# jianzhnie/ScaleRL

Measured on NVIDIA H100. Metric: learner_frames_per_sec, higher is better.
Workload: dtype bf16

## Files before the change

scalerl_b200/csrc/common.cuh:

```cuda
#pragma once
#include <cuda_runtime.h>
#include <cuda_bf16.h>
#include <stdint.h>
#include "wgmma.cuh"

#define SRL_DEVINL __device__ __forceinline__

#ifndef SRL_SPIN_LIMIT
#define SRL_SPIN_LIMIT (1u << 24)
#endif

namespace srl {

SRL_DEVINL uint32_t smem_u32(const void* p) { return static_cast<uint32_t>(__cvta_generic_to_shared(p)); }

SRL_DEVINL void mbar_init(uint64_t* bar, uint32_t count) {
  asm volatile("mbarrier.init.shared::cta.b64 [%0], %1;" ::"r"(smem_u32(bar)), "r"(count) : "memory");
}
SRL_DEVINL void mbar_fence_init() { asm volatile("fence.mbarrier_init.release.cluster;" ::: "memory"); }
SRL_DEVINL void mbar_arrive(uint64_t* bar) {
  asm volatile("{\n\t.reg .b64 st;\n\tmbarrier.arrive.shared::cta.b64 st, [%0];\n\t}" ::"r"(smem_u32(bar)) : "memory");
}
SRL_DEVINL void mbar_arrive_expect_tx(uint64_t* bar, uint32_t bytes) {
  asm volatile("{\n\t.reg .b64 st;\n\tmbarrier.arrive.expect_tx.shared::cta.b64 st, [%0], %1;\n\t}" ::"r"(smem_u32(bar)), "r"(bytes)
// ... 111 lines not shown

SRL_DEVINL uint64_t make_smem_desc(uint32_t saddr, uint32_t lbo_bytes, uint32_t sbo_bytes) {
  uint64_t d = 0;
  d |= (uint64_t)((saddr & 0x3FFFF) >> 4);
  d |= (uint64_t)((lbo_bytes >> 4) & 0x3FFF) << 16;
  d |= (uint64_t)((sbo_bytes >> 4) & 0x3FFF) << 32;
  d |= (uint64_t)1 << 62;
  return d;
}
SRL_DEVINL uint64_t make_smem_desc_sw64(uint32_t saddr, uint32_t lbo_bytes, uint32_t sbo_bytes) {
  return (make_smem_desc(saddr, lbo_bytes, sbo_bytes) & ~((uint64_t)3 << 62)) | ((uint64_t)2 << 62);
}

SRL_DEVINL uint32_t swz128(uint32_t row, uint32_t chunk) { return row * 128u + ((chunk ^ (row & 7u)) << 4); }
SRL_DEVINL uint32_t swz64(uint32_t row, uint32_t chunk) { return row * 64u + ((chunk ^ ((row >> 1) & 3u)) << 4); }

SRL_DEVINL uint32_t pack_bf16x2(float lo, float hi) {
  __nv_bfloat162 v = __floats2bfloat162_rn(lo, hi);
  return *reinterpret_cast<uint32_t*>(&v);
}
SRL_DEVINL float bf16_lo(uint32_t v) { return __uint_as_float(v << 16); }
SRL_DEVINL float bf16_hi(uint32_t v) { return __uint_as_float(v & 0xFFFF0000u); }

SRL_DEVINL void red_add_v4(float* addr, float a, float b, float c, float d) {
  asm volatile("red.global.add.v4.f32 [%0], {%1, %2, %3, %4};" ::"l"(addr), "f"(a), "f"(b), "f"(c), "f"(d) : "memory");
}
SRL_DEVINL void red_add_16(float* dst, const float (&v)[16], float scale = 1.0f) {
#pragma unroll
  for (int j = 0; j < 16; j += 4) red_add_v4(dst + j, v[j] * scale, v[j + 1] * scale, v[j + 2] * scale, v[j + 3] * scale);
}

SRL_DEVINL int ld_action(const int64_t* p, int A) {
  const long long a = __ldg(reinterpret_cast<const long long*>(p));
  return a < 0 ? 0 : (a >= A ? A - 1 : (int)a);
}

SRL_DEVINL uint4 philox4x32_10(uint4 c, uint2 k) {
#pragma unroll
  for (int r = 0; r < 10; ++r) {
    const uint32_t hi0 = __umulhi(0xD2511F53u, c.x), lo0 = 0xD2511F53u * c.x;
    const uint32_t hi1 = __umulhi(0xCD9E8D57u, c.z), lo1 = 0xCD9E8D57u * c.z;
    c = make_uint4(hi1 ^ c.y ^ k.x, lo1, hi0 ^ c.w ^ k.y, lo0);
    k.x += 0x9E3779B9u; k.y += 0xBB67AE85u;
  }
  return c;
}
// ... 14 lines not shown
```

scalerl_b200/csrc/encoder.cu:

```cuda
#include "encoder_problems.cuh"
#include "tma_problems.cuh"
#include "res_problems.cuh"
#include "enc_fused.cuh"
#include "kernels.h"
#include <stdio.h>
#include <stdlib.h>

namespace srl {

constexpr int PACK_BLOCKS_FK = 256, PACK_BLOCKS_FD = 256, PACK_BLOCKS_CONV = 288;
SRL_DEVINL void pack_store(bf16* __restrict__ out, bf16* __restrict__ out_lo, int64_t i, float v) {
  const bf16 hi = __float2bfloat16_rn(v);
  out[i] = hi;
  if (out_lo) out_lo[i] = __float2bfloat16_rn(v - __bfloat162float(hi));
}
SRL_DEVINL void pack_store2(bf16* __restrict__ out, bf16* __restrict__ out_lo, int64_t i, float v0, float v1) {
  const bf16 h0 = __float2bfloat16_rn(v0), h1 = __float2bfloat16_rn(v1);
  *reinterpret_cast<uint32_t*>(out + i) = pack_bf16x2(v0, v1);
  if (out_lo) *reinterpret_cast<uint32_t*>(out_lo + i) = pack_bf16x2(v0 - __bfloat162float(h0), v1 - __bfloat162float(h1));
}
__global__ void __launch_bounds__(256) pack_weights_kernel(ParamPtrs p, bf16* __restrict__ out, bf16* __restrict__ out_lo, int skip_w1k) {
  pdl_wait(2);
  __shared__ __align__(16) float tile[64 * 99];
  const int t = threadIdx.x, b = blockIdx.x;
// ... 303 lines not shown
                            const StepStreams& S, bool fused_front) {
  if (frames <= 0) return cudaSuccess;
  if ((mode != 0 && mode != 1) || !maps.valid) return cudaErrorInvalidValue;
  const int sp = mode;
  if (sp && !buf.lo.wpack) return cudaErrorInvalidValue;
  const cudaStream_t st = S.main;
  if (fused_front && !sp && (reinterpret_cast<uintptr_t>(obs) & 15) == 0) {
    EncFusedParams q{obs, p.w1, p.b1, p.w2, p.b2, buf.xs, buf.hi.a1, buf.hi.a2, frames, buf.NF};
    S.b(PS_ENC_FUSED); SRL_TRY(enc_fused_fwd_launch(q, kPersistentCtas, st)); S.e(PS_ENC_FUSED);
    SRL_TRY(S.join(LANE_PACK));
  } else {
  S.b(PS_S2D); SRL_TRY(launch_s2d(obs, frames, buf.xs, st, p.w1, buf.hi.wpack + WPack::W1K, sp ? buf.lo.wpack + WPack::W1K : nullptr)); S.e(PS_S2D);
  { RConv1Fwd::Params q{maps.xs_w, maps.hi.w1k, maps.lo.w1k, p.b1, buf.hi.a1, buf.lo.a1, frames, buf.NF};
    S.b(PS_CONV1_FWD); SRL_TRY(res_fwd_launch<RConv1Fwd>(q, cdiv(frames * 441, 128), kPersistentCtas, st, sp)); S.e(PS_CONV1_FWD); }
  SRL_TRY(S.join(LANE_PACK));
  { RConv2Fwd::Params q{maps.hi.a1p0_w, maps.hi.a1p1_w, maps.hi.w2k, maps.lo.a1p0_w, maps.lo.a1p1_w, maps.lo.w2k, p.b2, buf.hi.a2, buf.lo.a2, frames};
    S.b(PS_CONV2_FWD); SRL_TRY(res_fwd_launch<RConv2Fwd>(q, cdiv(frames * 100, 128), kPersistentCtas, st, sp)); S.e(PS_CONV2_FWD); }
  }
  { RConv3Fwd::Params q{maps.hi.a2_w, maps.hi.w3k, maps.lo.a2_w, maps.lo.w3k, p.b3, buf.hi.a3, buf.lo.a3, frames};
    S.b(PS_CONV3_FWD); SRL_TRY(res_fwd_launch<RConv3Fwd>(q, cdiv(frames * 81, 128), kPersistentCtas, st, sp)); S.e(PS_CONV3_FWD); }
  { TFcFwd::Params q{maps.hi.a3m128, maps.hi.wfk, maps.lo.a3m128, maps.lo.wfk, buf.hpart, frames};
    static_assert(TFcFwd::SPLITS == FC_SPLITS, "split count");
    S.b(PS_FC_FWD);
    if (sp) SRL_TRY((igemm_tma_launch<TFcFwd, 1>(q, dim3(cdiv(frames, 128), 8 * FC_SPLITS), st)));
    else SRL_TRY((igemm_tma_launch<TFcFwd, 0>(q, dim3(cdiv(frames, 128), 8 * FC_SPLITS), st)));
    S.e(PS_FC_FWD); }
  return cudaSuccess;
}

cudaError_t encoder_backward(int frames, const EncoderBuffers& buf, const ParamPtrs& g, const TmaMaps& maps, int mode,
                             const StepStreams& S, BwdParts parts, bool a3t_done) {
  if (frames <= 0) return cudaSuccess;
  if ((mode != 0 && mode != 1) || !maps.valid) return cudaErrorInvalidValue;
  const int sp = mode;
  if (sp && !buf.lo.wpack) return cudaErrorInvalidValue;
  const bool do_fc = parts & BWD_FC, do_conv = parts & BWD_CONV;
  const cudaStream_t st = S.main, s1 = S.lane(LANE_FC_WGRAD), s2 = S.lane(LANE_CONV3_WGRAD), s3 = S.lane(LANE_CONV2_WGRAD);
  if (do_fc) {
    SRL_TRY(S.fork(LANE_FC_WGRAD));
    { const bool native = !sp && buf.a3t != nullptr;
      S.b(PS_FC_WGRAD);
      if (native) {
        if (!a3t_done) SRL_TRY(launch_a3_transpose(buf.hi.a3, buf.a3t, frames, s1));
        TFcWgradN::Params q{maps.hi.dhm64, maps.a3tm64, g.wf, g.bf, frames};
        SRL_TRY((igemm_tma_launch<TFcWgradN, 0>(q, dim3(1, 4 * (TFcWgradN::NCT + 1)), s1)));
      } else {
        TFcWgrad::Params q{maps.hi.dhm64, maps.hi.a3m64, maps.lo.dhm64, maps.lo.a3m64, g.wf, g.bf, frames};
        if (sp) SRL_TRY((igemm_tma_launch<TFcWgrad, 1>(q, dim3(1, 4 * 50), s1))); else SRL_TRY((igemm_tma_launch<TFcWgrad, 0>(q, dim3(1, 4 * 50), s1)));
      }
      S.e(PS_FC_WGRAD); }
    { TFcDgrad::Params q{maps.hi.dhm128, maps.hi.wfd, maps.lo.dhm128, maps.lo.wfd, buf.hi.a3, buf.hi.da3, buf.lo.da3, frames};
      S.b(PS_FC_DGRAD);
      if (sp) SRL_TRY((igemm_tma_launch<TFcDgrad, 1>(q, dim3(cdiv(frames, 128), 49), st))); else SRL_TRY((igemm_tma_launch<TFcDgrad, 0>(q, dim3(cdiv(frames, 128), 49), st)));
      S.e(PS_FC_DGRAD); }
    if (!do_conv) SRL_TRY(S.join(LANE_FC_WGRAD));
  }
  if (!do_conv) return cudaSuccess;
  SRL_TRY(S.fork(LANE_CONV3_WGRAD));
  float* part3 = buf.wgrad_part;
  float* part2 = part3 + (size_t)WG_PART_CTAS * WSP_W3;
  float* part1 = part2 + (size_t)WG_PART_CTAS * WSP_W2;
  int n3 = 0, n2 = 0, n1 = 0;
  { RConv3Wgrad::Params q{maps.hi.a2_w, maps.hi.da3g_b, maps.lo.a2_w, maps.lo.da3g_b, part3, frames * 81, 0};
    S.b(PS_CONV3_WGRAD); SRL_TRY(res_wgrad_launch<RConv3Wgrad>(q, side_wgrad_ctas(), s2, &n3, sp)); S.e(PS_CONV3_WGRAD); }
  if (!S.collapsed) SRL_TRY(launch_wgrad_reduce<WgradReduce3>(part3, n3, g.w3, g.b3, s2));
  { RConv3Dgrad::Params q{maps.hi.da3g_w, maps.hi.w3d, maps.lo.da3g_w, maps.lo.w3d, buf.hi.a2, buf.hi.da2, buf.lo.da2, frames};
    S.b(PS_CONV3_DGRAD); SRL_TRY(res_fwd_launch<RConv3Dgrad>(q, cdiv(frames * 81, 128), bwd_ctas(), st, sp)); S.e(PS_CONV3_DGRAD); }
  SRL_TRY(S.fork(LANE_CONV2_WGRAD));
  { RConv2Wgrad::Params q{maps.hi.a1p0_w, maps.hi.a1p1_w, maps.hi.da2g_b, maps.lo.a1p0_w, maps.lo.a1p1_w, maps.lo.da2g_b, part2, frames * 100, 0};
    S.b(PS_CONV2_WGRAD); SRL_TRY(res_wgrad_launch<RConv2Wgrad>(q, side_wgrad_ctas(), s3, &n2, sp)); S.e(PS_CONV2_WGRAD); }
  if (!S.collapsed) SRL_TRY(launch_wgrad_reduce<WgradReduce2>(part2, n2, g.w2, g.b2, s3));
  { RConv2Dgrad::Params q{maps.hi.da2g_w, maps.hi.w2d, maps.lo.da2g_w, maps.lo.w2d, buf.hi.a1, buf.hi.da1, buf.lo.da1, frames, buf.NF};
    S.b(PS_CONV2_DGRAD); SRL_TRY(res_fwd_launch<RConv2Dgrad>(q, cdiv(frames * 100, 128), bwd_ctas(), st, sp)); S.e(PS_CONV2_DGRAD); }
  { RConv1Wgrad::Params q{maps.xs_w, maps.hi.da1g_b, maps.lo.da1g_b, part1, frames * 441, 0};
    S.b(PS_CONV1_WGRAD); SRL_TRY(res_wgrad_launch<RConv1Wgrad>(q, bwd_ctas(), st, &n1, sp)); S.e(PS_CONV1_WGRAD); }
  S.b(PS_WGRAD_FINALIZE);
// ... 14 lines not shown
```

scalerl_b200/csrc/igemm_res.cuh:

```cuda
#pragma once
#include "igemm_tma.cuh"

namespace srl {

constexpr int RES_THREADS = 384;
constexpr int RES_PRODUCER_REGS = 40, RES_CONSUMER_REGS = 232;
constexpr int RES_MAX_TAPS = 10;


template <int N, int ROWB, class F>
SRL_DEVINL void wg_acc_stage_bf16(const float (&d)[2][N / 2], uint8_t* buf, int wt, int bar, F f) {
  static_assert(ROWB % 16 == 0 && ROWB >= 2 * N, "16-byte aligned rows that hold N bf16");
  const int w = wt >> 5, l = wt & 31;
  named_bar(bar, 128);
#pragma unroll
  for (int h = 0; h < 2; ++h)
#pragma unroll
    for (int i = 0; i < N / 2; i += 2) {
      const int row = 64 * h + 16 * w + (l >> 2) + 8 * ((i >> 1) & 1), col = 8 * (i >> 2) + 2 * (l & 3);
      *reinterpret_cast<uint32_t*>(buf + row * ROWB + col * 2) = pack_bf16x2(f(col, d[h][i]), f(col + 1, d[h][i + 1]));
    }
  named_bar(bar, 128);
}
template <class P, int SPLIT>
struct ResFwdCfg {
  static constexpr int ALO = (SPLIT && P::A_LO) ? 1 : 0;
  static constexpr int WIN_BYTES = ((P::WROWS * 128 + 1023) / 1024) * 1024;
  static constexpr int IN_HI_BYTES = P::NWIN * WIN_BYTES;
  static constexpr int IN_BYTES = IN_HI_BYTES * (1 + ALO);
  static constexpr int W_HI_BYTES = P::NT * P::BN * 128;
  static constexpr int W_BYTES = W_HI_BYTES * (1 + SPLIT);
  static constexpr bool TILE_EPI = P::TILE_ROWB > 0 && !SPLIT;
  static constexpr int TILE_IMG_BYTES = 128 * P::TILE_ROWB > WG_IMG_BYTES ? 128 * P::TILE_ROWB : WG_IMG_BYTES;
  static constexpr bool IMG1 = !TILE_EPI && W_BYTES + IN_BYTES + 2 * WG_IMG_BYTES + 1024 + 256 > 232448;
  static constexpr int IMG_BYTES = TILE_EPI ? TILE_IMG_BYTES : IMG1 ? WG_IMG_BYTES / 2 : WG_IMG_BYTES;
  static constexpr int FIT = fit_stages(SPLIT ? P::SPLIT_STAGES : P::STAGES, W_BYTES + 2 * IMG_BYTES + 1024 + 256, IN_BYTES);
  static constexpr int STAGES = FIT > 1 ? FIT & ~1 : 1;
  static constexpr int SMEM_BYTES = W_BYTES + STAGES * IN_BYTES + 2 * IMG_BYTES + 1024 + 256;
  static_assert(SMEM_BYTES <= 232448, "shared memory budget (227 KB)");
  static_assert(W_BYTES % 1024 == 0, "weight block alignment");
  static_assert(P::BN == 32 || P::BN == 64 || P::BN == 128, "MMA N");
};

template <class P, int SPLIT>
__global__ void __launch_bounds__(RES_THREADS, 1) res_fwd_kernel(const __grid_constant__ typename P::Params p) {
  using C = ResFwdCfg<P, SPLIT>;
// ... 362 lines not shown
```

scalerl_b200/csrc/igemm_tma.cuh:

```cuda
#pragma once
#include <cuda.h>
#include "common.cuh"
#include "kernels.h"

namespace srl {

SRL_DEVINL void tma_prefetch_desc(const CUtensorMap* m) {
  asm volatile("prefetch.tensormap [%0];" ::"l"(reinterpret_cast<uint64_t>(m)) : "memory");
}
SRL_DEVINL void tma_load_2d(void* dst, const CUtensorMap* m, uint64_t* bar, int c0, int c1) {
  asm volatile("cp.async.bulk.tensor.2d.shared::cluster.global.mbarrier::complete_tx::bytes [%0], [%1, {%3, %4}], [%2];"
               ::"r"(smem_u32(dst)), "l"(reinterpret_cast<uint64_t>(m)), "r"(smem_u32(bar)), "r"(c0), "r"(c1) : "memory");
}
SRL_DEVINL void tma_load_3d(void* dst, const CUtensorMap* m, uint64_t* bar, int c0, int c1, int c2) {
  asm volatile("cp.async.bulk.tensor.3d.shared::cluster.global.mbarrier::complete_tx::bytes [%0], [%1, {%3, %4, %5}], [%2];"
               ::"r"(smem_u32(dst)), "l"(reinterpret_cast<uint64_t>(m)), "r"(smem_u32(bar)), "r"(c0), "r"(c1), "r"(c2) : "memory");
}
SRL_DEVINL void tma_load_4d(void* dst, const CUtensorMap* m, uint64_t* bar, int c0, int c1, int c2, int c3) {
  asm volatile("cp.async.bulk.tensor.4d.shared::cluster.global.mbarrier::complete_tx::bytes [%0], [%1, {%3, %4, %5, %6}], [%2];"
               ::"r"(smem_u32(dst)), "l"(reinterpret_cast<uint64_t>(m)), "r"(smem_u32(bar)), "r"(c0), "r"(c1), "r"(c2), "r"(c3)
               : "memory");
}
SRL_DEVINL void tma_load_5d(void* dst, const CUtensorMap* m, uint64_t* bar, int c0, int c1, int c2, int c3, int c4) {
  asm volatile("cp.async.bulk.tensor.5d.shared::cluster.global.mbarrier::complete_tx::bytes [%0], [%1, {%3, %4, %5, %6, %7}], [%2];"
               ::"r"(smem_u32(dst)), "l"(reinterpret_cast<uint64_t>(m)), "r"(smem_u32(bar)), "r"(c0), "r"(c1), "r"(c2), "r"(c3), "r"(c4)
               : "memory");
}

constexpr int IGT_THREADS = 288;

template <class P, int SPLIT = 0>
struct TmaCfg {
  static constexpr int KROWS = P::A_MN ? P::KROWS : 64;
  static constexpr int A_BYTES = P::A_MN ? 2 * KROWS * 128 : 128 * 128;
  static constexpr int B_BLOCKS = (P::BN + 63) / 64;
  static constexpr int B_BYTES = P::B_MN ? B_BLOCKS * KROWS * 128 : P::BN * 128;
  static constexpr int HALF_BYTES = A_BYTES + B_BYTES;
  static constexpr int STAGE_BYTES = HALF_BYTES * (1 + SPLIT);
  static constexpr int NB = P::BN / 2;
  static constexpr int STAGES = fit_stages(P::STAGES, 2 * WG_IMG_BYTES + 1024 + 256, STAGE_BYTES);
  static constexpr int SMEM_BYTES = STAGES * STAGE_BYTES + 2 * WG_IMG_BYTES + 1024 + 256;
  static_assert(SMEM_BYTES <= 232448, "shared memory budget (227 KB)");
  static_assert(NB == 32 || NB == 64 || NB == 128, "MMA N per warpgroup");
  static constexpr int MMAS = P::A_MN ? KROWS / 16 : 4;
  static_assert(A_BYTES % 1024 == 0 && B_BYTES % 1024 == 0, "operand tiles must keep 1024 B alignment (SWIZZLE_128B atoms)");
  static_assert(P::A_MN == P::B_MN, "mixed majors are not used");
  static_assert(KROWS % 16 == 0, "contraction rows per stage must be a multiple of MMA K = 16");
};

template <class P, int SPLIT>
SRL_DEVINL void igt_epilogue(const typename P::Params& p, int tm, int ty, int row, int c0, float (&v)[16]) {
  if constexpr (SPLIT) P::template epilogue16<1>(p, tm, ty, row, c0, v); else P::epilogue16(p, tm, ty, row, c0, v);
}
template <class P, int SPLIT>
SRL_DEVINL void igt_epilogue(const typename P::Params& p, int tm, int ty, int row, int c0, float (&v)[16], const uint4 (&pre)[2]) {
  if constexpr (SPLIT) P::template epilogue16<1>(p, tm, ty, row, c0, v, pre); else P::epilogue16(p, tm, ty, row, c0, v, pre);
}

template <class P, int SPLIT = 0>
__global__ void __launch_bounds__(IGT_THREADS) igemm_tma_kernel(const __grid_constant__ typename P::Params p) {
  using C = TmaCfg<P, SPLIT>;
  extern __shared__ uint8_t smem_raw[];
  uint8_t* smem = reinterpret_cast<uint8_t*>((reinterpret_cast<uintptr_t>(smem_raw) + 1023) & ~uintptr_t(1023));
  float* img = reinterpret_cast<float*>(smem + C::STAGES * C::STAGE_BYTES);
  uint64_t* bars = reinterpret_cast<uint64_t*>(smem + C::STAGES * C::STAGE_BYTES + 2 * WG_IMG_BYTES);
  uint64_t* full = bars;
  uint64_t* empty = bars + C::STAGES;

  const int tid = threadIdx.x;
  const int warp = tid >> 5;
  const int tm = blockIdx.x, ty = blockIdx.y;
  const int nkb = P::num_kblocks(p, tm, ty);

  if constexpr (P::ZERO_INIT) {
    if (P::zero_cta(ty)) {
      uint4* z = reinterpret_cast<uint4*>(smem);
      for (int i = tid; i < C::STAGES * C::STAGE_BYTES / 16; i += IGT_THREADS) z[i] = make_uint4(0, 0, 0, 0);
    }
    __syncthreads();
    for (int s = 0; s < C::STAGES; ++s) P::init_smem(p, tm, ty, smem + s * C::STAGE_BYTES, tid);
    fence_proxy_async_smem();
  }
  if (warp == 8 && (tid & 31) == 0) {
    for (int s = 0; s < C::STAGES; ++s) { mbar_init(&full[s], 1); mbar_init(&empty[s], 8); }
    mbar_fence_init();
    P::prefetch(p);
  }
  __syncthreads();
  pdl_wait(P::KID);
  if (tid == 256) pdl_launch();

  if (warp == 8) {
    const uint32_t leader = elect_one_sync();
    for (int kb = 0; kb < nkb; ++kb) {
      const int s = kb % C::STAGES;
      mbar_wait(&empty[s], ((kb / C::STAGES) & 1) ^ 1);
      if (leader) {
        uint8_t* sA = smem + s * C::STAGE_BYTES;
        if constexpr (SPLIT) P::issue_split(p, tm, ty, kb, sA, C::A_BYTES, C::HALF_BYTES, &full[s]);
        else P::issue(p, tm, ty, kb, sA, sA + C::A_BYTES, &full[s]);
      }
      __syncwarp();
    }
  } else {
    const int g = warp >> 2, wt = tid & 127;
    constexpr int NB = C::NB;
    uint4 pre[P::PREFETCH ? NB / 16 : 1][2];
    if constexpr (P::PREFETCH) {
#pragma unroll
      for (int c = 0; c < NB / 16; ++c) P::prefetch16(p, tm, ty, wt, g * NB + c * 16, pre[c]);
    }
    float acc[2][NB / 2];
#pragma unroll
    for (int h = 0; h < 2; ++h)
#pragma unroll
// ... 10 lines not shown
      wg_fence();
#pragma unroll
      for (int k = 0; k < C::MMAS; ++k) {
        const uint64_t ad = ad0 + (uint64_t)(k * ASTEP), bd = bd0 + (uint64_t)(k * BSTEP);
        wg_mma128<NB, P::A_MN ? 1 : 0, P::B_MN ? 1 : 0>(acc, ad, A_HI, bd, (kb | k) != 0);
        if constexpr (SPLIT) {
          wg_mma128<NB, P::A_MN ? 1 : 0, P::B_MN ? 1 : 0>(acc, ad, A_HI, bd + (uint64_t)(C::HALF_BYTES / 16), 1);
          wg_mma128<NB, P::A_MN ? 1 : 0, P::B_MN ? 1 : 0>(acc, ad + (uint64_t)(C::HALF_BYTES / 16), A_HI, bd, 1);
        }
      }
      wg_commit();
      if constexpr (C::STAGES > 1) {
        wg_wait_prev();
        __syncwarp();
        if (kb > 0 && (tid & 31) == 0) mbar_arrive(&empty[(kb - 1) % C::STAGES]);
      } else {
        wg_wait_all();
        __syncwarp();
        if ((tid & 31) == 0) mbar_arrive(&empty[s]);
      }
    }
    wg_wait_all();
    wg_fence_regs(acc[0]); wg_fence_regs(acc[1]);
    float* my_img = img + g * (WG_IMG_BYTES / 4);
#pragma unroll
    for (int c = 0; c < NB / 16; ++c) {
      float v[16];
      wg_acc_row16<NB>(acc, c, my_img, wt, 2 + g, v);
      if constexpr (P::PREFETCH) igt_epilogue<P, SPLIT>(p, tm, ty, wt, g * NB + c * 16, v, pre[c]);
      else igt_epilogue<P, SPLIT>(p, tm, ty, wt, g * NB + c * 16, v);
    }
  }
}

template <class P, int SPLIT = 0>
cudaError_t igemm_tma_launch(const typename P::Params& p, dim3 grid, cudaStream_t stream) {
  using C = TmaCfg<P, SPLIT>;
  if (grid.x == 0 || grid.y == 0) return cudaSuccess;
  static PerDeviceOnce once;
  { cudaError_t e = ensure_max_dynamic_smem(once, igemm_tma_kernel<P, SPLIT>, C::SMEM_BYTES); if (e != cudaSuccess) return e; }
  return launch_chain(igemm_tma_kernel<P, SPLIT>, grid, dim3(IGT_THREADS), C::SMEM_BYTES, stream, p);
}

}
```

scalerl_b200/csrc/lstm.cu:

```cuda
#include <cstring>
#include <new>
#include "tma_problems.cuh"
#include "kernels.h"
#include "errors.h"
#include "../../include/scalerl_b200.h"

namespace srl {

struct LGemmK {
  static constexpr int KID = 34;
  static constexpr bool PREFETCH = false;
  static constexpr int BN = 64, STAGES = 4, KROWS = 64;
  static constexpr bool A_MN = false, B_MN = false, ZERO_INIT = false;
  struct Params { SRL_TMAP a; SRL_TMAP b; float* C; int M, nkb, ldc, a_row0, c_row0; };
  SRL_DEVINL static void prefetch(const Params& p) { tma_prefetch_desc(&p.a); tma_prefetch_desc(&p.b); }
  SRL_DEVINL static int num_kblocks(const Params& p, int, int) { return p.nkb; }
  SRL_DEVINL static void issue(const Params& p, int tm, int ty, int kb, uint8_t* sA, uint8_t* sB, uint64_t* bar) {
    mbar_arrive_expect_tx(bar, 128 * 128 + 64 * 128);
    tma_load_2d(sA, &p.a, bar, kb * 64, p.a_row0 + tm * 128);
    tma_load_2d(sB, &p.b, bar, kb * 64, ty * 64);
  }
  SRL_DEVINL static void epilogue16(const Params& p, int tm, int ty, int row, int c0, float (&v)[16]) {
    const int m = tm * 128 + row;
    if (m >= p.M) return;
    float4* o = reinterpret_cast<float4*>(p.C + (size_t)(p.c_row0 + m) * p.ldc + ty * 64 + c0);
#pragma unroll
    for (int j = 0; j < 4; ++j) o[j] = make_float4(v[4 * j], v[4 * j + 1], v[4 * j + 2], v[4 * j + 3]);
  }
};
struct LGemmMN {
  static constexpr int KID = 35;
  static constexpr bool PREFETCH = false;
  static constexpr int BN = 64, STAGES = 4, KROWS = 64;
  static constexpr bool A_MN = true, B_MN = true, ZERO_INIT = false;
  struct Params { SRL_TMAP a; SRL_TMAP b; float* C; int R, ldc; };
  SRL_DEVINL static void prefetch(const Params& p) { tma_prefetch_desc(&p.a); tma_prefetch_desc(&p.b); }
  SRL_DEVINL static int num_kblocks(const Params& p, int, int) { return (p.R + 63) >> 6; }
  SRL_DEVINL static void init_smem(const Params&, int, int, uint8_t*, int, int) {}
  SRL_DEVINL static void issue(const Params& p, int tm, int ty, int kb, uint8_t* sA, uint8_t* sB, uint64_t* bar) {
    mbar_arrive_expect_tx(bar, 3 * 64 * 128);
    tma_load_2d(sA, &p.a, bar, tm * 128, kb * 64);
    tma_load_2d(sA + KROWS * 128, &p.a, bar, tm * 128 + 64, kb * 64);
    tma_load_2d(sB, &p.b, bar, ty * 64, kb * 64);
  }
  SRL_DEVINL static void epilogue16(const Params& p, int tm, int ty, int row, int c0, float (&v)[16]) {
    float4* o = reinterpret_cast<float4*>(p.C + (size_t)(tm * 128 + row) * p.ldc + ty * 64 + c0);
#pragma unroll
    for (int j = 0; j < 4; ++j) o[j] = make_float4(v[4 * j], v[4 * j + 1], v[4 * j + 2], v[4 * j + 3]);
  }
};

SRL_DEVINL float sigmoidf_(float x) { return 1.0f / (1.0f + expf(-x)); }

__global__ void lstm_pad_bf16_kernel(const float* __restrict__ x, int rows, int H, int Hp, __nv_bfloat16* __restrict__ out) {
  const int64_t i = (int64_t)blockIdx.x * blockDim.x + threadIdx.x;
  if (i >= (int64_t)rows * Hp) return;
  const int r = (int)(i / Hp), j = (int)(i - (int64_t)r * Hp);
// ... 690 lines not shown
```

scalerl_b200/csrc/tma_problems.cuh:

```cuda
#pragma once
#include "igemm_tma.cuh"
#include "encoder_problems.cuh"

namespace srl {

#define SRL_TMAP alignas(64) CUtensorMap

struct TFcFwd {
  static constexpr int KID = 31;
  static constexpr bool PREFETCH = false;
  static constexpr int BN = 64, STAGES = 4, SPLITS = 4;
  static constexpr bool A_MN = false, B_MN = false, ZERO_INIT = false;
  static constexpr int KROWS = 64;
  struct Params { SRL_TMAP a3m; SRL_TMAP w; SRL_TMAP a3m_lo; SRL_TMAP w_lo; float* out; int M; };
  SRL_DEVINL static void prefetch(const Params& p) { tma_prefetch_desc(&p.a3m); tma_prefetch_desc(&p.w); }
  SRL_DEVINL static int kb_begin(int split) { return (49 * split) / SPLITS; }
  SRL_DEVINL static void issue_split(const Params& p, int tm, int ty, int kb, uint8_t* st, int a_bytes, int half, uint64_t* bar) {
    const int k = (kb_begin(ty % SPLITS) + kb) * 64;
    mbar_arrive_expect_tx(bar, 2 * (128 * 128 + 64 * 128));
    tma_load_2d(st, &p.a3m, bar, k, tm * 128);
    tma_load_2d(st + a_bytes, &p.w, bar, k, (ty / SPLITS) * 64);
    tma_load_2d(st + half, &p.a3m_lo, bar, k, tm * 128);
    tma_load_2d(st + half + a_bytes, &p.w_lo, bar, k, (ty / SPLITS) * 64);
  }
  template <int SPLIT>
  SRL_DEVINL static void epilogue16(const Params& p, int tm, int ty, int row, int c0, float (&v)[16]) { epilogue16(p, tm, ty, row, c0, v); }
  SRL_DEVINL static int num_kblocks(const Params&, int, int ty) { const int sp = ty % SPLITS; return kb_begin(sp + 1) - kb_begin(sp); }
  SRL_DEVINL static void issue(const Params& p, int tm, int ty, int kb, uint8_t* sA, uint8_t* sB, uint64_t* bar) {
    const int k = (kb_begin(ty % SPLITS) + kb) * 64;
    mbar_arrive_expect_tx(bar, 128 * 128 + 64 * 128);
    tma_load_2d(sA, &p.a3m, bar, k, tm * 128);
    tma_load_2d(sB, &p.w, bar, k, (ty / SPLITS) * 64);
  }
  SRL_DEVINL static void epilogue16(const Params& p, int tm, int ty, int row, int c0, float (&v)[16]) {
    const int m = tm * 128 + row;
    if (m >= p.M) return;
    float4* o = reinterpret_cast<float4*>(p.out + ((size_t)(ty % SPLITS) * p.M + m) * 512 + (ty / SPLITS) * 64 + c0);
#pragma unroll
    for (int j = 0; j < 4; ++j) o[j] = make_float4(v[4 * j], v[4 * j + 1], v[4 * j + 2], v[4 * j + 3]);
  }
};

struct TFcDgrad {
  static constexpr int KID = 32;
  static constexpr bool PREFETCH = true;
  static constexpr int BN = 64, STAGES = 4;
  static constexpr bool A_MN = false, B_MN = false, ZERO_INIT = false;
  static constexpr int KROWS = 64;
  struct Params { SRL_TMAP dhm; SRL_TMAP w; SRL_TMAP dhm_lo; SRL_TMAP w_lo; const bf16* a3; bf16* da3; bf16* da3_lo; int M; };
  SRL_DEVINL static void prefetch(const Params& p) { tma_prefetch_desc(&p.dhm); tma_prefetch_desc(&p.w); }
  SRL_DEVINL static int num_kblocks(const Params&, int, int) { return 8; }
  SRL_DEVINL static void issue_split(const Params& p, int tm, int ty, int kb, uint8_t* st, int a_bytes, int half, uint64_t* bar) {
    mbar_arrive_expect_tx(bar, 2 * (128 * 128 + 64 * 128));
    tma_load_2d(st, &p.dhm, bar, kb * 64, tm * 128);
    tma_load_2d(st + a_bytes, &p.w, bar, kb * 64, ty * 64);
    tma_load_2d(st + half, &p.dhm_lo, bar, kb * 64, tm * 128);
    tma_load_2d(st + half + a_bytes, &p.w_lo, bar, kb * 64, ty * 64);
  }
  SRL_DEVINL static void issue(const Params& p, int tm, int ty, int kb, uint8_t* sA, uint8_t* sB, uint64_t* bar) {
    mbar_arrive_expect_tx(bar, 128 * 128 + 64 * 128);
    tma_load_2d(sA, &p.dhm, bar, kb * 64, tm * 128);
    tma_load_2d(sB, &p.w, bar, kb * 64, ty * 64);
  }
  SRL_DEVINL static void prefetch16(const Params& p, int tm, int ty, int row, int c0, uint4 (&mk)[2]) {
    const int m = tm * 128 + row;
    if (m < p.M) ld_mask16(p.a3 + (size_t)m * 3136 + ty * 64 + c0, mk);
  }
  SRL_DEVINL static void epilogue16(const Params& p, int tm, int ty, int row, int c0, float (&v)[16], const uint4 (&mk)[2]) {
    epilogue16<0>(p, tm, ty, row, c0, v, mk);
  }
  template <int SPLIT>
  SRL_DEVINL static void epilogue16(const Params& p, int tm, int ty, int row, int c0, float (&v)[16], const uint4 (&mk)[2]) {
    const int m = tm * 128 + row;
    if (m >= p.M) return;
    relu_mask16_pre(mk, v);
    const size_t o = ((size_t)m * 81 + (ty / 7) * 9 + ty % 7) * 64 + c0;
    store_bf16x16(p.da3 + o, v);
    if constexpr (SPLIT) {
      float r[16];
#pragma unroll
      for (int j = 0; j < 16; ++j) r[j] = v[j] - __bfloat162float(__float2bfloat16_rn(v[j]));
      store_bf16x16(p.da3_lo + o, r);
    }
  }
};

SRL_DEVINL void fill_ones(uint8_t* dst, int bytes, int tid) {
  uint4* q = reinterpret_cast<uint4*>(dst);
  for (int i = tid; i < bytes / 16; i += IGT_THREADS) q[i] = make_uint4(0x3F803F80u, 0x3F803F80u, 0x3F803F80u, 0x3F803F80u);
}

struct TFcWgrad {
  static constexpr int KID = 33;
  static constexpr bool PREFETCH = false;
  static constexpr int BN = 64, STAGES = 4, KROWS = 64;
  static constexpr bool A_MN = true, B_MN = true, ZERO_INIT = true;
  struct Params { SRL_TMAP dhm; SRL_TMAP a3m; SRL_TMAP dhm_lo; SRL_TMAP a3m_lo; float* dw; float* db; int M; };
  SRL_DEVINL static void prefetch(const Params& p) { tma_prefetch_desc(&p.dhm); tma_prefetch_desc(&p.a3m); }
  SRL_DEVINL static void issue_split(const Params& p, int, int ty, int kb, uint8_t* st, int a_bytes, int half, uint64_t* bar) {
    const int hw = ty >> 2, j0 = (ty & 3) * 128;
    mbar_arrive_expect_tx(bar, (hw < 49 ? 6 : 4) * 64 * 128);
    tma_load_2d(st, &p.dhm, bar, j0, kb * 64);
    tma_load_2d(st + KROWS * 128, &p.dhm, bar, j0 + 64, kb * 64);
    tma_load_2d(st + half, &p.dhm_lo, bar, j0, kb * 64);
    tma_load_2d(st + half + KROWS * 128, &p.dhm_lo, bar, j0 + 64, kb * 64);
    if (hw < 49) {
      tma_load_2d(st + a_bytes, &p.a3m, bar, hw * 64, kb * 64);
      tma_load_2d(st + half + a_bytes, &p.a3m_lo, bar, hw * 64, kb * 64);
    }
  }
  template <int SPLIT>
  SRL_DEVINL static void epilogue16(const Params& p, int tm, int ty, int row, int c0, float (&v)[16]) { epilogue16(p, tm, ty, row, c0, v); }
  SRL_DEVINL static bool zero_cta(int) { return true; }
  SRL_DEVINL static int num_kblocks(const Params& p, int, int) { return (p.M + 63) >> 6; }
  SRL_DEVINL static void init_smem(const Params&, int, int ty, uint8_t* stage, int tid) {
    if ((ty >> 2) == 49) fill_ones(stage + 2 * KROWS * 128, KROWS * 128, tid);
  }
  SRL_DEVINL static void issue(const Params& p, int, int ty, int kb, uint8_t* sA, uint8_t* sB, uint64_t* bar) {
    const int hw = ty >> 2, j0 = (ty & 3) * 128;
    mbar_arrive_expect_tx(bar, (hw < 49 ? 3 : 2) * 64 * 128);
    tma_load_2d(sA, &p.dhm, bar, j0, kb * 64);
    tma_load_2d(sA + KROWS * 128, &p.dhm, bar, j0 + 64, kb * 64);
    if (hw < 49) tma_load_2d(sB, &p.a3m, bar, hw * 64, kb * 64);
  }
  SRL_DEVINL static void epilogue16(const Params& p, int, int ty, int row, int c0, float (&v)[16]) {
    const int j = (ty & 3) * 128 + row, hw = ty >> 2;
    if (hw < 49) {
#pragma unroll
      for (int jj = 0; jj < 16; ++jj) p.dw[(size_t)j * 3136 + (c0 + jj) * 49 + hw] = v[jj];
    } else if (c0 == 0) {
      p.db[j] = v[0];
    }
  }
};

struct TFcWgradN {
  static constexpr int KID = 36;
  static constexpr bool PREFETCH = false;
  static constexpr int BN = 256, STAGES = 4, KROWS = 64, NCT = 13;
  static constexpr bool A_MN = true, B_MN = true, ZERO_INIT = true;
  struct Params { SRL_TMAP dhm; SRL_TMAP a3tm; float* dw; float* db; int M; };
  SRL_DEVINL static void prefetch(const Params& p) { tma_prefetch_desc(&p.dhm); tma_prefetch_desc(&p.a3tm); }
  SRL_DEVINL static bool zero_cta(int ty) { return (ty >> 2) == NCT; }
  SRL_DEVINL static int num_kblocks(const Params& p, int, int) { return (p.M + 63) >> 6; }
  SRL_DEVINL static void init_smem(const Params&, int, int ty, uint8_t* stage, int tid) {
    if ((ty >> 2) == NCT) fill_ones(stage + 2 * KROWS * 128, KROWS * 128, tid);
  }
  SRL_DEVINL static void issue(const Params& p, int, int ty, int kb, uint8_t* sA, uint8_t* sB, uint64_t* bar) {
    const int ct = ty >> 2, j0 = (ty & 3) * 128;
    const int nb = ct < NCT ? (ct == NCT - 1 ? 1 : 4) : 0;
    mbar_arrive_expect_tx(bar, (2 + nb) * 64 * 128);
    tma_load_2d(sA, &p.dhm, bar, j0, kb * 64);
    tma_load_2d(sA + KROWS * 128, &p.dhm, bar, j0 + 64, kb * 64);
    for (int q = 0; q < nb; ++q) tma_load_2d(sB + q * KROWS * 128, &p.a3tm, bar, ct * 256 + q * 64, kb * 64);
  }
  SRL_DEVINL static void epilogue16(const Params& p, int, int ty, int row, int c0, float (&v)[16]) {
    const int j = (ty & 3) * 128 + row, ct = ty >> 2, col = ct * 256 + c0;
    if (ct < NCT) {
      if (col < 3136) {
        float4* d = reinterpret_cast<float4*>(p.dw + (size_t)j * 3136 + col);
#pragma unroll
        for (int q = 0; q < 4; ++q) d[q] = make_float4(v[4 * q], v[4 * q + 1], v[4 * q + 2], v[4 * q + 3]);
      }
    } else if (c0 == 0) {
      p.db[j] = v[0];
    }
  }
};

}
```

Before: 2.615 million.

## Make FC forward/dgrad GEMMs persistent tile loops and stage epilogues through smem

Converts the FC forward and FC dgrad TMA GEMMs into persistent kernels. A single producer warp streams k-blocks for many tiles through one mbarrier ring, and the two consumer warpgroups alternate whole tiles, each using the full BN width. This lets one tile's epilogue overlap the next tile's mainloop and removes per-CTA launch and prologue cost. Epilogues now stage accumulators through shared memory so global stores are coalesced 16-byte rows. The FC wgrad kernel also stages its output through the idle ring buffer. The changes add register pressure (full-width accumulators per warpgroup) and more complex barrier handoff, which risks stalls or lower occupancy.

Measured after the change: 2.643 million (median of 6 runs). +1.1%, better.

```diff
diff --git a/scalerl_b200/csrc/common.cuh b/scalerl_b200/csrc/common.cuh
--- a/scalerl_b200/csrc/common.cuh
+++ b/scalerl_b200/csrc/common.cuh
@@ -157,6 +157,33 @@
 SRL_DEVINL float bf16_lo(uint32_t v) { return __uint_as_float(v << 16); }
 SRL_DEVINL float bf16_hi(uint32_t v) { return __uint_as_float(v & 0xFFFF0000u); }
 
+template <int N, int ROWB, class F>
+SRL_DEVINL void wg_acc_stage_bf16(const float (&d)[2][N / 2], uint8_t* buf, int wt, int bar, F f) {
+  static_assert(ROWB % 16 == 0 && ROWB >= 2 * N, "16-byte aligned rows that hold N bf16");
+  const int w = wt >> 5, l = wt & 31;
+  named_bar(bar, 128);
+#pragma unroll
+  for (int h = 0; h < 2; ++h)
+#pragma unroll
+    for (int i = 0; i < N / 2; i += 2) {
+      const int row = 64 * h + 16 * w + (l >> 2) + 8 * ((i >> 1) & 1), col = 8 * (i >> 2) + 2 * (l & 3);
+      *reinterpret_cast<uint32_t*>(buf + row * ROWB + col * 2) = pack_bf16x2(f(col, d[h][i]), f(col + 1, d[h][i + 1]));
+    }
+  named_bar(bar, 128);
+}
+template <int N, int ROWB>
+SRL_DEVINL void wg_acc_stage_f32(const float (&d)[N / 2], uint8_t* buf, int wt, int bar) {
+  static_assert(ROWB % 16 == 0 && ROWB >= 4 * N, "16-byte aligned rows that hold N floats");
+  const int w = wt >> 5, l = wt & 31;
+  named_bar(bar, 128);
+#pragma unroll
+  for (int i = 0; i < N / 2; i += 2) {
+    const int row = 16 * w + (l >> 2) + 8 * ((i >> 1) & 1), col = 8 * (i >> 2) + 2 * (l & 3);
+    *reinterpret_cast<float2*>(buf + row * ROWB + col * 4) = make_float2(d[i], d[i + 1]);
+  }
+  named_bar(bar, 128);
+}
+
 SRL_DEVINL void red_add_v4(float* addr, float a, float b, float c, float d) {
   asm volatile("red.global.add.v4.f32 [%0], {%1, %2, %3, %4};" ::"l"(addr), "f"(a), "f"(b), "f"(c), "f"(d) : "memory");
 }
diff --git a/scalerl_b200/csrc/encoder.cu b/scalerl_b200/csrc/encoder.cu
--- a/scalerl_b200/csrc/encoder.cu
+++ b/scalerl_b200/csrc/encoder.cu
@@ -349,8 +349,8 @@
   { TFcFwd::Params q{maps.hi.a3m128, maps.hi.wfk, maps.lo.a3m128, maps.lo.wfk, buf.hpart, frames};
     static_assert(TFcFwd::SPLITS == FC_SPLITS, "split count");
     S.b(PS_FC_FWD);
-    if (sp) SRL_TRY((igemm_tma_launch<TFcFwd, 1>(q, dim3(cdiv(frames, 128), 8 * FC_SPLITS), st)));
-    else SRL_TRY((igemm_tma_launch<TFcFwd, 0>(q, dim3(cdiv(frames, 128), 8 * FC_SPLITS), st)));
+    if (sp) SRL_TRY((igemm_tma_launch_tiles<TFcFwd, 1>(q, cdiv(frames, 128) * 8 * FC_SPLITS, kPersistentCtas, st)));
+    else SRL_TRY((igemm_tma_launch_tiles<TFcFwd, 0>(q, cdiv(frames, 128) * 8 * FC_SPLITS, kPersistentCtas, st)));
     S.e(PS_FC_FWD); }
   return cudaSuccess;
 }
@@ -378,7 +378,8 @@
       S.e(PS_FC_WGRAD); }
     { TFcDgrad::Params q{maps.hi.dhm128, maps.hi.wfd, maps.lo.dhm128, maps.lo.wfd, buf.hi.a3, buf.hi.da3, buf.lo.da3, frames};
       S.b(PS_FC_DGRAD);
-      if (sp) SRL_TRY((igemm_tma_launch<TFcDgrad, 1>(q, dim3(cdiv(frames, 128), 49), st))); else SRL_TRY((igemm_tma_launch<TFcDgrad, 0>(q, dim3(cdiv(frames, 128), 49), st)));
+      if (sp) SRL_TRY((igemm_tma_launch_tiles<TFcDgrad, 1>(q, cdiv(frames, 128) * 49, kPersistentCtas, st)));
+      else SRL_TRY((igemm_tma_launch_tiles<TFcDgrad, 0>(q, cdiv(frames, 128) * 49, kPersistentCtas, st)));
       S.e(PS_FC_DGRAD); }
     if (!do_conv) SRL_TRY(S.join(LANE_FC_WGRAD));
   }
diff --git a/scalerl_b200/csrc/igemm_res.cuh b/scalerl_b200/csrc/igemm_res.cuh
--- a/scalerl_b200/csrc/igemm_res.cuh
+++ b/scalerl_b200/csrc/igemm_res.cuh
@@ -8,20 +8,6 @@
 constexpr int RES_MAX_TAPS = 10;
 
 
-template <int N, int ROWB, class F>
-SRL_DEVINL void wg_acc_stage_bf16(const float (&d)[2][N / 2], uint8_t* buf, int wt, int bar, F f) {
-  static_assert(ROWB % 16 == 0 && ROWB >= 2 * N, "16-byte aligned rows that hold N bf16");
-  const int w = wt >> 5, l = wt & 31;
-  named_bar(bar, 128);
-#pragma unroll
-  for (int h = 0; h < 2; ++h)
-#pragma unroll
-    for (int i = 0; i < N / 2; i += 2) {
-      const int row = 64 * h + 16 * w + (l >> 2) + 8 * ((i >> 1) & 1), col = 8 * (i >> 2) + 2 * (l & 3);
-      *reinterpret_cast<uint32_t*>(buf + row * ROWB + col * 2) = pack_bf16x2(f(col, d[h][i]), f(col + 1, d[h][i + 1]));
-    }
-  named_bar(bar, 128);
-}
 template <class P, int SPLIT>
 struct ResFwdCfg {
   static constexpr int ALO = (SPLIT && P::A_LO) ? 1 : 0;
diff --git a/scalerl_b200/csrc/igemm_tma.cuh b/scalerl_b200/csrc/igemm_tma.cuh
--- a/scalerl_b200/csrc/igemm_tma.cuh
+++ b/scalerl_b200/csrc/igemm_tma.cuh
@@ -37,7 +37,7 @@
   static constexpr int B_BYTES = P::B_MN ? B_BLOCKS * KROWS * 128 : P::BN * 128;
   static constexpr int HALF_BYTES = A_BYTES + B_BYTES;
   static constexpr int STAGE_BYTES = HALF_BYTES * (1 + SPLIT);
-  static constexpr int NB = P::BN / 2;
+  static constexpr int NB = P::PERSISTENT ? P::BN : P::BN / 2;
   static constexpr int STAGES = fit_stages(P::STAGES, 2 * WG_IMG_BYTES + 1024 + 256, STAGE_BYTES);
   static constexpr int SMEM_BYTES = STAGES * STAGE_BYTES + 2 * WG_IMG_BYTES + 1024 + 256;
   static_assert(SMEM_BYTES <= 232448, "shared memory budget (227 KB)");
@@ -45,6 +45,7 @@
   static constexpr int MMAS = P::A_MN ? KROWS / 16 : 4;
   static_assert(A_BYTES % 1024 == 0 && B_BYTES % 1024 == 0, "operand tiles must keep 1024 B alignment (SWIZZLE_128B atoms)");
   static_assert(P::A_MN == P::B_MN, "mixed majors are not used");
+  static_assert(!P::PERSISTENT || (!P::A_MN && !P::ZERO_INIT && STAGES > 1), "tile loop: K-major operands, a ring of two or more stages");
   static_assert(KROWS % 16 == 0, "contraction rows per stage must be a multiple of MMA K = 16");
 };
 
@@ -55,6 +56,93 @@
 template <class P, int SPLIT>
 SRL_DEVINL void igt_epilogue(const typename P::Params& p, int tm, int ty, int row, int c0, float (&v)[16], const uint4 (&pre)[2]) {
   if constexpr (SPLIT) P::template epilogue16<1>(p, tm, ty, row, c0, v, pre); else P::epilogue16(p, tm, ty, row, c0, v, pre);
+}
+
+template <class P, int SPLIT>
+SRL_DEVINL void igt_tile_producer(const typename P::Params& p, uint8_t* smem, uint64_t* full, uint64_t* empty) {
+  using C = TmaCfg<P, SPLIT>;
+  const uint32_t leader = elect_one_sync();
+  const int ntiles = P::num_tiles(p);
+  int q = 0;
+  for (int t = blockIdx.x; t < ntiles; t += gridDim.x) {
+    int tm, ty;
+    P::tile(p, t, tm, ty);
+    const int nkb = P::num_kblocks(p, tm, ty);
+    for (int kb = 0; kb < nkb; ++kb, ++q) {
+      const int s = q % C::STAGES;
+      mbar_wait(&empty[s], ((q / C::STAGES) & 1) ^ 1);
+      if (leader) {
+        uint8_t* sA = smem + s * C::STAGE_BYTES;
+        if constexpr (SPLIT) P::issue_split(p, tm, ty, kb, sA, C::A_BYTES, C::HALF_BYTES, &full[s]);
+        else P::issue(p, tm, ty, kb, sA, sA + C::A_BYTES, &full[s]);
+      }
+      __syncwarp();
+    }
+  }
+}
+
+template <class P, int SPLIT>
+SRL_DEVINL void igt_tile_consumer(const typename P::Params& p, uint8_t* smem, float* img, uint64_t* full, uint64_t* empty, int g, int tid) {
+  using C = TmaCfg<P, SPLIT>;
+  constexpr int NB = C::NB;
+  constexpr uint32_t A_HI = 64 * 128 / 16;
+  const int wt = tid & 127, ntiles = P::num_tiles(p);
+  float* my_img = img + g * (WG_IMG_BYTES / 4);
+  int q = 0, it = 0;
+  for (int t = blockIdx.x; t < ntiles; t += gridDim.x, ++it) {
+    int tm, ty;
+    P::tile(p, t, tm, ty);
+    const int nkb = P::num_kblocks(p, tm, ty);
+    if ((it & 1) != g) { q += nkb; continue; }
+    const bool next = t + (int)gridDim.x < ntiles;
+    uint4 pre[P::PREFETCH ? NB / 16 : 1][2];
+    if constexpr (P::PREFETCH) {
+      if constexpr (SPLIT) {
+#pragma unroll
+        for (int c = 0; c < NB / 16; ++c) P::prefetch16(p, tm, ty, wt, c * 16, pre[c]);
+      } else {
+        P::prefetch_tile(p, tm, ty, wt, pre);
+      }
+    }
+    if (it > 0) named_bar(4 + g, 256);
+    float acc[2][NB / 2];
+    for (int kb = 0; kb < nkb; ++kb, ++q) {
+      const int s = q % C::STAGES;
+      mbar_wait(&full[s], (q / C::STAGES) & 1);
+      if (kb == nkb - 1 && next) asm volatile("bar.arrive %0, 256;" ::"r"(5 - g) : "memory");
+      const uint32_t a0 = smem_u32(smem + s * C::STAGE_BYTES);
+      const uint64_t ad0 = make_smem_desc(a0, 16, 1024), bd0 = make_smem_desc(a0 + C::A_BYTES, 16, 1024);
+      wg_fence();
+#pragma unroll
+      for (int k = 0; k < C::MMAS; ++k) {
+        const uint64_t ad = ad0 + (uint64_t)(2 * k), bd = bd0 + (uint64_t)(2 * k);
+        wg_mma128<NB, 0, 0>(acc, ad, A_HI, bd, (kb | k) != 0);
+        if constexpr (SPLIT) {
+          wg_mma128<NB, 0, 0>(acc, ad, A_HI, bd + (uint64_t)(C::HALF_BYTES / 16), 1);
+          wg_mma128<NB, 0, 0>(acc, ad + (uint64_t)(C::HALF_BYTES / 16), A_HI, bd, 1);
+        }
+      }
+      wg_commit();
+      wg_wait_prev();
+      __syncwarp();
+      if (kb > 0 && (tid & 31) == 0) mbar_arrive(&empty[(q - 1) % C::STAGES]);
+    }
+    wg_wait_all();
+    wg_fence_regs(acc[0]); wg_fence_regs(acc[1]);
+    __syncwarp();
+    if ((tid & 31) == 0) mbar_arrive(&empty[(q - 1) % C::STAGES]);
+    if constexpr (SPLIT) {
+#pragma unroll
+      for (int c = 0; c < NB / 16; ++c) {
+        float v[16];
+        wg_acc_row16<NB>(acc, c, my_img, wt, 2 + g, v);
+        if constexpr (P::PREFETCH) igt_epilogue<P, SPLIT>(p, tm, ty, wt, c * 16, v, pre[c]);
+        else igt_epilogue<P, SPLIT>(p, tm, ty, wt, c * 16, v);
+      }
+    } else {
+      P::epilogue_tile(p, tm, ty, wt, acc, reinterpret_cast<uint8_t*>(my_img), 2 + g, pre);
+    }
+  }
 }
 
 template <class P, int SPLIT = 0>
@@ -70,7 +158,7 @@
   const int tid = threadIdx.x;
   const int warp = tid >> 5;
   const int tm = blockIdx.x, ty = blockIdx.y;
-  const int nkb = P::num_kblocks(p, tm, ty);
+  const int nkb = P::PERSISTENT ? 0 : P::num_kblocks(p, tm, ty);
 
   if constexpr (P::ZERO_INIT) {
     if (P::zero_cta(ty)) {
@@ -82,7 +170,7 @@
     fence_proxy_async_smem();
   }
   if (warp == 8 && (tid & 31) == 0) {
-    for (int s = 0; s < C::STAGES; ++s) { mbar_init(&full[s], 1); mbar_init(&empty[s], 8); }
+    for (int s = 0; s < C::STAGES; ++s) { mbar_init(&full[s], 1); mbar_init(&empty[s], P::PERSISTENT ? 4 : 8); }
     mbar_fence_init();
     P::prefetch(p);
   }
@@ -90,7 +178,10 @@
   pdl_wait(P::KID);
   if (tid == 256) pdl_launch();
 
-  if (warp == 8) {
+  if constexpr (P::PERSISTENT) {
+    if (warp == 8) igt_tile_producer<P, SPLIT>(p, smem, full, empty);
+    else igt_tile_consumer<P, SPLIT>(p, smem, img, full, empty, warp >> 2, tid);
+  } else if (warp == 8) {
     const uint32_t leader = elect_one_sync();
     for (int kb = 0; kb < nkb; ++kb) {
       const int s = kb % C::STAGES;
@@ -147,13 +238,22 @@
     }
     wg_wait_all();
     wg_fence_regs(acc[0]); wg_fence_regs(acc[1]);
-    float* my_img = img + g * (WG_IMG_BYTES / 4);
-#pragma unroll
-    for (int c = 0; c < NB / 16; ++c) {
-      float v[16];
-      wg_acc_row16<NB>(acc, c, my_img, wt, 2 + g, v);
-      if constexpr (P::PREFETCH) igt_epilogue<P, SPLIT>(p, tm, ty, wt, g * NB + c * 16, v, pre[c]);
-      else igt_epilogue<P, SPLIT>(p, tm, ty, wt, g * NB + c * 16, v);
+    if constexpr (P::RING_ROWB > 0 && !SPLIT) {
+      static_assert(2 * 128 * P::RING_ROWB <= C::STAGES * C::STAGE_BYTES && P::RING_ROWB >= 4 * NB, "staged tile fits the ring");
+      named_bar(4, 256);
+      uint8_t* blk = smem + g * 128 * P::RING_ROWB;
+      wg_acc_stage_f32<NB, P::RING_ROWB>(acc[0], blk, wt, 2 + g);
+      wg_acc_stage_f32<NB, P::RING_ROWB>(acc[1], blk + 64 * P::RING_ROWB, wt, 2 + g);
+      P::epilogue_ring(p, tm, ty, g, wt, blk);
+    } else {
+      float* my_img = img + g * (WG_IMG_BYTES / 4);
+#pragma unroll
+      for (int c = 0; c < NB / 16; ++c) {
+        float v[16];
+        wg_acc_row16<NB>(acc, c, my_img, wt, 2 + g, v);
+        if constexpr (P::PREFETCH) igt_epilogue<P, SPLIT>(p, tm, ty, wt, g * NB + c * 16, v, pre[c]);
+        else igt_epilogue<P, SPLIT>(p, tm, ty, wt, g * NB + c * 16, v);
+      }
     }
   }
 }
@@ -161,10 +261,22 @@
 template <class P, int SPLIT = 0>
 cudaError_t igemm_tma_launch(const typename P::Params& p, dim3 grid, cudaStream_t stream) {
   using C = TmaCfg<P, SPLIT>;
+  static_assert(!P::PERSISTENT, "tile-loop problems launch through igemm_tma_launch_tiles");
   if (grid.x == 0 || grid.y == 0) return cudaSuccess;
   static PerDeviceOnce once;
   { cudaError_t e = ensure_max_dynamic_smem(once, igemm_tma_kernel<P, SPLIT>, C::SMEM_BYTES); if (e != cudaSuccess) return e; }
   return launch_chain(igemm_tma_kernel<P, SPLIT>, grid, dim3(IGT_THREADS), C::SMEM_BYTES, stream, p);
 }
 
-}
+template <class P, int SPLIT = 0>
+cudaError_t igemm_tma_launch_tiles(const typename P::Params& p, int ntiles, int max_ctas, cudaStream_t stream) {
+  using C = TmaCfg<P, SPLIT>;
+  static_assert(P::PERSISTENT, "one-tile-per-CTA problems launch through igemm_tma_launch");
+  if (ntiles <= 0) return cudaSuccess;
+  static PerDeviceOnce once;
+  { cudaError_t e = ensure_max_dynamic_smem(once, igemm_tma_kernel<P, SPLIT>, C::SMEM_BYTES); if (e != cudaSuccess) return e; }
+  const int rounds = (ntiles + max_ctas - 1) / max_ctas;
+  return launch_chain(igemm_tma_kernel<P, SPLIT>, dim3((ntiles + rounds - 1) / rounds), dim3(IGT_THREADS), C::SMEM_BYTES, stream, p);
+}
+
+}
diff --git a/scalerl_b200/csrc/lstm.cu b/scalerl_b200/csrc/lstm.cu
--- a/scalerl_b200/csrc/lstm.cu
+++ b/scalerl_b200/csrc/lstm.cu
@@ -11,7 +11,8 @@
   static constexpr int KID = 34;
   static constexpr bool PREFETCH = false;
   static constexpr int BN = 64, STAGES = 4, KROWS = 64;
-  static constexpr bool A_MN = false, B_MN = false, ZERO_INIT = false;
+  static constexpr bool A_MN = false, B_MN = false, ZERO_INIT = false, PERSISTENT = false;
+  static constexpr int RING_ROWB = 0;
   struct Params { SRL_TMAP a; SRL_TMAP b; float* C; int M, nkb, ldc, a_row0, c_row0; };
   SRL_DEVINL static void prefetch(const Params& p) { tma_prefetch_desc(&p.a); tma_prefetch_desc(&p.b); }
   SRL_DEVINL static int num_kblocks(const Params& p, int, int) { return p.nkb; }
@@ -32,7 +33,8 @@
   static constexpr int KID = 35;
   static constexpr bool PREFETCH = false;
   static constexpr int BN = 64, STAGES = 4, KROWS = 64;
-  static constexpr bool A_MN = true, B_MN = true, ZERO_INIT = false;
+  static constexpr bool A_MN = true, B_MN = true, ZERO_INIT = false, PERSISTENT = false;
+  static constexpr int RING_ROWB = 0;
   struct Params { SRL_TMAP a; SRL_TMAP b; float* C; int R, ldc; };
   SRL_DEVINL static void prefetch(const Params& p) { tma_prefetch_desc(&p.a); tma_prefetch_desc(&p.b); }
   SRL_DEVINL static int num_kblocks(const Params& p, int, int) { return (p.R + 63) >> 6; }
diff --git a/scalerl_b200/csrc/tma_problems.cuh b/scalerl_b200/csrc/tma_problems.cuh
--- a/scalerl_b200/csrc/tma_problems.cuh
+++ b/scalerl_b200/csrc/tma_problems.cuh
@@ -10,11 +10,13 @@
   static constexpr int KID = 31;
   static constexpr bool PREFETCH = false;
   static constexpr int BN = 64, STAGES = 4, SPLITS = 4;
-  static constexpr bool A_MN = false, B_MN = false, ZERO_INIT = false;
+  static constexpr bool A_MN = false, B_MN = false, ZERO_INIT = false, PERSISTENT = true;
   static constexpr int KROWS = 64;
   struct Params { SRL_TMAP a3m; SRL_TMAP w; SRL_TMAP a3m_lo; SRL_TMAP w_lo; float* out; int M; };
   SRL_DEVINL static void prefetch(const Params& p) { tma_prefetch_desc(&p.a3m); tma_prefetch_desc(&p.w); }
   SRL_DEVINL static int kb_begin(int split) { return (49 * split) / SPLITS; }
+  SRL_DEVINL static int num_tiles(const Params& p) { return ((p.M + 127) >> 7) * 8 * SPLITS; }
+  SRL_DEVINL static void tile(const Params&, int t, int& tm, int& ty) { tm = t / (8 * SPLITS); ty = t - tm * (8 * SPLITS); }
   SRL_DEVINL static void issue_split(const Params& p, int tm, int ty, int kb, uint8_t* st, int a_bytes, int half, uint64_t* bar) {
     const int k = (kb_begin(ty % SPLITS) + kb) * 64;
     mbar_arrive_expect_tx(bar, 2 * (128 * 128 + 64 * 128));
@@ -39,17 +41,35 @@
 #pragma unroll
     for (int j = 0; j < 4; ++j) o[j] = make_float4(v[4 * j], v[4 * j + 1], v[4 * j + 2], v[4 * j + 3]);
   }
+  static constexpr int TILE_ROWB = 288;
+  SRL_DEVINL static void prefetch_tile(const Params&, int, int, int, uint4 (&)[1][2]) {}
+  SRL_DEVINL static void epilogue_tile(const Params& p, int tm, int ty, int wt, const float (&acc)[2][BN / 2], uint8_t* img, int bar,
+                                       const uint4 (&)[1][2]) {
+    static_assert(64 * TILE_ROWB <= WG_IMG_BYTES, "a staged half fits the warpgroup's hand-off buffer");
+    float* out = p.out + (size_t)(ty % SPLITS) * p.M * 512 + (ty / SPLITS) * 64;
+#pragma unroll
+    for (int h = 0; h < 2; ++h) {
+      wg_acc_stage_f32<BN, TILE_ROWB>(acc[h], img, wt, bar);
+#pragma unroll
+      for (int s = 0; s < 8; ++s) {
+        const int e = s * 128 + wt, r = e >> 4, k = e & 15, m = tm * 128 + 64 * h + r;
+        if (m < p.M) *reinterpret_cast<uint4*>(out + (size_t)m * 512 + k * 4) = *reinterpret_cast<const uint4*>(img + r * TILE_ROWB + k * 16);
+      }
+    }
+  }
 };
 
 struct TFcDgrad {
   static constexpr int KID = 32;
   static constexpr bool PREFETCH = true;
   static constexpr int BN = 64, STAGES = 4;
-  static constexpr bool A_MN = false, B_MN = false, ZERO_INIT = false;
+  static constexpr bool A_MN = false, B_MN = false, ZERO_INIT = false, PERSISTENT = true;
   static constexpr int KROWS = 64;
   struct Params { SRL_TMAP dhm; SRL_TMAP w; SRL_TMAP dhm_lo; SRL_TMAP w_lo; const bf16* a3; bf16* da3; bf16* da3_lo; int M; };
   SRL_DEVINL static void prefetch(const Params& p) { tma_prefetch_desc(&p.dhm); tma_prefetch_desc(&p.w); }
   SRL_DEVINL static int num_kblocks(const Params&, int, int) { return 8; }
+  SRL_DEVINL static int num_tiles(const Params& p) { return ((p.M + 127) >> 7) * 49; }
+  SRL_DEVINL static void tile(const Params&, int t, int& tm, int& ty) { tm = t / 49; ty = t - tm * 49; }
   SRL_DEVINL static void issue_split(const Params& p, int tm, int ty, int kb, uint8_t* st, int a_bytes, int half, uint64_t* bar) {
     mbar_arrive_expect_tx(bar, 2 * (128 * 128 + 64 * 128));
     tma_load_2d(st, &p.dhm, bar, kb * 64, tm * 128);
@@ -66,8 +86,26 @@
     const int m = tm * 128 + row;
     if (m < p.M) ld_mask16(p.a3 + (size_t)m * 3136 + ty * 64 + c0, mk);
   }
-  SRL_DEVINL static void epilogue16(const Params& p, int tm, int ty, int row, int c0, float (&v)[16], const uint4 (&mk)[2]) {
-    epilogue16<0>(p, tm, ty, row, c0, v, mk);
+  static constexpr int TILE_ROWB = 144;
+  SRL_DEVINL static void prefetch_tile(const Params& p, int tm, int ty, int wt, uint4 (&mk)[BN / 16][2]) {
+#pragma unroll
+    for (int s = 0; s < 8; ++s) {
+      const int e = s * 128 + wt, m = tm * 128 + (e >> 3);
+      if (m < p.M) mk[s >> 1][s & 1] = ldg16(p.a3 + (size_t)m * 3136 + ty * 64 + (e & 7) * 8);
+    }
+  }
+  SRL_DEVINL static void epilogue_tile(const Params& p, int tm, int ty, int wt, const float (&acc)[2][BN / 2], uint8_t* img, int bar,
+                                       const uint4 (&mk)[BN / 16][2]) {
+    wg_acc_stage_bf16<BN, TILE_ROWB>(acc, img, wt, bar, [](int, float v) { return v; });
+    bf16* out = p.da3 + ((ty / 7) * 9 + ty % 7) * 64;
+#pragma unroll
+    for (int s = 0; s < 8; ++s) {
+      const int e = s * 128 + wt, q = e >> 3, k = e & 7, m = tm * 128 + q;
+      if (m >= p.M) continue;
+      const uint4 x = *reinterpret_cast<const uint4*>(img + q * TILE_ROWB + k * 16), w = mk[s >> 1][s & 1];
+      *reinterpret_cast<uint4*>(out + (size_t)m * 81 * 64 + k * 8) =
+          make_uint4(relu_mask_bf16x2(x.x, w.x), relu_mask_bf16x2(x.y, w.y), relu_mask_bf16x2(x.z, w.z), relu_mask_bf16x2(x.w, w.w));
+    }
   }
   template <int SPLIT>
   SRL_DEVINL static void epilogue16(const Params& p, int tm, int ty, int row, int c0, float (&v)[16], const uint4 (&mk)[2]) {
@@ -94,7 +132,8 @@
   static constexpr int KID = 33;
   static constexpr bool PREFETCH = false;
   static constexpr int BN = 64, STAGES = 4, KROWS = 64;
-  static constexpr bool A_MN = true, B_MN = true, ZERO_INIT = true;
+  static constexpr bool A_MN = true, B_MN = true, ZERO_INIT = true, PERSISTENT = false;
+  static constexpr int RING_ROWB = 0;
   struct Params { SRL_TMAP dhm; SRL_TMAP a3m; SRL_TMAP dhm_lo; SRL_TMAP a3m_lo; float* dw; float* db; int M; };
   SRL_DEVINL static void prefetch(const Params& p) { tma_prefetch_desc(&p.dhm); tma_prefetch_desc(&p.a3m); }
   SRL_DEVINL static void issue_split(const Params& p, int, int ty, int kb, uint8_t* st, int a_bytes, int half, uint64_t* bar) {
@@ -138,7 +177,8 @@
   static constexpr int KID = 36;
   static constexpr bool PREFETCH = false;
   static constexpr int BN = 256, STAGES = 4, KROWS = 64, NCT = 13;
-  static constexpr bool A_MN = true, B_MN = true, ZERO_INIT = true;
+  static constexpr bool A_MN = true, B_MN = true, ZERO_INIT = true, PERSISTENT = false;
+  static constexpr int RING_ROWB = 544;
   struct Params { SRL_TMAP dhm; SRL_TMAP a3tm; float* dw; float* db; int M; };
   SRL_DEVINL static void prefetch(const Params& p) { tma_prefetch_desc(&p.dhm); tma_prefetch_desc(&p.a3tm); }
   SRL_DEVINL static bool zero_cta(int ty) { return (ty >> 2) == NCT; }
@@ -166,6 +206,19 @@
       p.db[j] = v[0];
     }
   }
+  SRL_DEVINL static void epilogue_ring(const Params& p, int, int ty, int g, int wt, const uint8_t* blk) {
+    const int j0 = (ty & 3) * 128, ct = ty >> 2, col0 = ct * 256 + g * 128;
+    if (ct == NCT) {
+      if (g == 0) p.db[j0 + wt] = *reinterpret_cast<const float*>(blk + wt * RING_ROWB);
+      return;
+    }
+#pragma unroll 8
+    for (int s = 0; s < 32; ++s) {
+      const int e = s * 128 + wt, r = e >> 5, k = e & 31;
+      if (col0 + 4 * k < 3136)
+        *reinterpret_cast<uint4*>(p.dw + (size_t)(j0 + r) * 3136 + col0 + 4 * k) = *reinterpret_cast<const uint4*>(blk + r * RING_ROWB + k * 16);
+    }
+  }
 };
 
 }
```
